# IDEA-CCNL/Fengshenbang-LM

Hardware: AMD Instinct MI355X
Metric: tokens/sec Ziya-LLaMA-13B ZeRO-3 (higher is better)
Workload: dtype bf16; 1 GPU; model=Ziya-LLaMA-13B, global_batch=16, micro_batch=16, seq_len=2048, parallelism=zero3_dp1, activation_checkpointing=True, ckpt_skip_interval=4

## Files before the change

fengshen_amd/ops/csrc/flash_attn.hip:

```cpp

#include "common.h"

typedef __attribute__((ext_vector_type(8))) short bf16x8;
typedef __attribute__((ext_vector_type(4))) float f32x4;

#define FA_QBLK 128
#define FA_KVBLK 64
#define FA_WAVES 8
#define FA_VPAD 8
#define FB_T 32

constexpr int fa_dpad(int d) { return (d + 31) / 32 * 32; }
constexpr int fa_swb(int dp) {
  int need = 2 * dp, p = 128;
  while (p < need) p <<= 1;
  return p;
}

__device__ __forceinline__ int kswz(int row, int byte_in_row) {
  return byte_in_row ^ ((row & 7) << 4);
}

__device__ __forceinline__ unsigned int fa_hash(unsigned long long seed,
                                                unsigned long long idx) {
// ... 800 lines not shown
    b, h, sq, sk, scale, dth, ksc, seed, stream); break;
  switch (d) {
    FWD_CASE(40) FWD_CASE(64) FWD_CASE(80)
    FWD_CASE(96) FWD_CASE(128) FWD_CASE(160)
  }
#undef FWD_CASE
}

template <int D>
static void launch_bwd(bool causal, const void* q, const void* k,
                       const void* v, const void* o, const void* dout,
                       const float* lse, void* dq, void* dk, void* dv,
                       float* delta_ws, const int* klens, int b, int h,
                       int sq, int sk, float scale, unsigned int dth,
                       float ksc, unsigned long long seed,
                       hipStream_t stream) {
  const long rows = (long)b * h * sq;
  {
    long blocks = (rows + 3) / 4;
    if (blocks > 4096) blocks = 4096;
    hipLaunchKernelGGL((flash_delta_kernel<D>), dim3((unsigned)blocks),
                       dim3(256), 0, stream, (const bf16_t*)dout,
                       (const bf16_t*)o, delta_ws, rows);
  }
  dim3 gq((sq + FA_QBLK - 1) / FA_QBLK, h, b);
  dim3 gkv((sk + FA_WAVES * 16 - 1) / (FA_WAVES * 16), h, b);
  dim3 block(FA_WAVES * 64);
  if (causal) {
    hipLaunchKernelGGL((flash_attn_bwd_dq_kernel<D, true>), gq, block, 0,
                       stream, (const bf16_t*)q, (const bf16_t*)k,
                       (const bf16_t*)v, (const bf16_t*)dout, lse, delta_ws,
                       (bf16_t*)dq, klens, b, h, sq, sk, scale, dth, ksc,
                       seed);
    hipLaunchKernelGGL((flash_attn_bwd_dkv_kernel<D, true>), gkv, block, 0,
                       stream, (const bf16_t*)q, (const bf16_t*)k,
                       (const bf16_t*)v, (const bf16_t*)dout, lse, delta_ws,
                       (bf16_t*)dk, (bf16_t*)dv, klens, b, h, sq, sk, scale,
                       dth, ksc, seed);
  } else {
    hipLaunchKernelGGL((flash_attn_bwd_dq_kernel<D, false>), gq, block, 0,
                       stream, (const bf16_t*)q, (const bf16_t*)k,
                       (const bf16_t*)v, (const bf16_t*)dout, lse, delta_ws,
                       (bf16_t*)dq, klens, b, h, sq, sk, scale, dth, ksc,
                       seed);
    hipLaunchKernelGGL((flash_attn_bwd_dkv_kernel<D, false>), gkv, block, 0,
                       stream, (const bf16_t*)q, (const bf16_t*)k,
                       (const bf16_t*)v, (const bf16_t*)dout, lse, delta_ws,
                       (bf16_t*)dk, (bf16_t*)dv, klens, b, h, sq, sk, scale,
                       dth, ksc, seed);
  }
}

extern "C" void fs_flash_attn_bwd(const void* q, const void* k, const void* v,
                                  const void* o, const void* dout,
                                  const float* lse, void* dq, void* dk,
                                  void* dv, float* delta_ws, const int* klens,
                                  int b, int h, int sq, int sk, int d,
                                  int causal, float scale, float drop_p,
                                  unsigned long long seed,
                                  hipStream_t stream) {
  const unsigned int dth =
      (drop_p > 0.f) ? (unsigned int)(drop_p * 4294967296.0) : 0u;
  const float ksc = (drop_p > 0.f) ? 1.f / (1.f - drop_p) : 1.f;
#define BWD_CASE(DD) case DD: launch_bwd<DD>(causal, q, k, v, o, dout, lse, \
    dq, dk, dv, delta_ws, klens, b, h, sq, sk, scale, dth, ksc, seed, \
    stream); break;
  switch (d) {
    BWD_CASE(40) BWD_CASE(64) BWD_CASE(80)
    BWD_CASE(96) BWD_CASE(128) BWD_CASE(160)
  }
#undef BWD_CASE
}


#define V3_QBLK 256
#define V3_KVBLK 64

typedef __attribute__((ext_vector_type(16))) float f32x16;

struct FaStrides {
  long b, h, r;
};

template <int D>
__global__ __launch_bounds__(256)
void flash_delta_v3_kernel(const bf16_t* __restrict__ dO,
                           const bf16_t* __restrict__ O,
                           float* __restrict__ delta, FaStrides dos,
                           FaStrides os, int h, int s) {
  const int lane = threadIdx.x & 63;
  const int wid = threadIdx.x >> 6;
  const bf16_t* dob = dO + blockIdx.z * dos.b + blockIdx.y * dos.h;
  const bf16_t* ob = O + blockIdx.z * os.b + blockIdx.y * os.h;
  float* dl = delta + ((long)blockIdx.z * h + blockIdx.y) * s;
  for (int row = blockIdx.x * 4 + wid; row < s; row += gridDim.x * 4) {
    const bf16_t* dop = dob + row * dos.r;
    const bf16_t* op = ob + row * os.r;
    float sacc = 0.f;
    for (int i = lane * 2; i < D; i += 128) {
#pragma unroll
      for (int j = 0; j < 2; ++j)
        sacc += __bfloat162float(dop[i + j]) * __bfloat162float(op[i + j]);
    }
    sacc = wave_reduce_sum(sacc);
    if (lane == 0) dl[row] = sacc;
  }
}

template <int D, bool CAUSAL, bool HAS_DROP>
__global__ __launch_bounds__(FA_WAVES * 64)
void flash_attn_fwd_v3_kernel(const bf16_t* __restrict__ Q,
                              const bf16_t* __restrict__ K,
                              const bf16_t* __restrict__ V,
                              bf16_t* __restrict__ O,
                              float* __restrict__ LSE,
                              const int* __restrict__ klens,
                              FaStrides qs, FaStrides os,
                              int b, int h, int s, float scale,
                              unsigned int drop_thresh, float keep_scale,
                              unsigned long long drop_seed) {
  constexpr int NC = D / 16;
  constexpr int NTO = D / 32;
  constexpr int SWB = fa_swb(D);

  __shared__ char k_raw[2][V3_KVBLK * SWB];
  __shared__ short vt_lds[2][D][V3_KVBLK + FA_VPAD];

  const int lane = threadIdx.x & 63;
  const int wave = threadIdx.x >> 6;
  const int hi = lane >> 5;
  const int ln = lane & 31;
  const long bh = (long)blockIdx.z * h + blockIdx.y;
  const long qoff = blockIdx.z * qs.b + blockIdx.y * qs.h;
  const bf16_t* Qp = Q + qoff;
  const bf16_t* Kp = K + qoff;
  const bf16_t* Vp = V + qoff;
  bf16_t* Op = O + blockIdx.z * os.b + blockIdx.y * os.h;

  const int klen = CAUSAL ? s : min(klens ? klens[blockIdx.z] : s, s);

  const int q0w = blockIdx.x * V3_QBLK + wave * 32;
  const bool q_active = q0w < s;
  const int q0c = q_active ? q0w : s - 32;
  const int my_q = q0c + ln;

  bf16x8 q_frag[NC];
#pragma unroll
  for (int c = 0; c < NC; ++c) {
    bf16x8 raw = *reinterpret_cast<const bf16x8*>(
        Qp + (long)my_q * qs.r + c * 16 + hi * 8);
#pragma unroll
    for (int j = 0; j < 8; ++j) {
      unsigned short u = (unsigned short)raw[j];
      float f = __uint_as_float(((unsigned int)u) << 16) * scale;
      raw[j] = fa_bf16bits(f);
    }
    q_frag[c] = raw;
  }

  float m_run = -INFINITY, l_run = 0.f;
  f32x16 o_acc[NTO];
#pragma unroll
  for (int t = 0; t < NTO; ++t) {
#pragma unroll
    for (int r = 0; r < 16; ++r) o_acc[t][r] = 0.f;
  }

  int n_kv_tiles;
  if (CAUSAL) {
    const int q_hi_row = min(blockIdx.x * V3_QBLK + V3_QBLK, s) - 1;
    n_kv_tiles = (q_hi_row / V3_KVBLK) + 1;
  } else {
    n_kv_tiles = (klen + V3_KVBLK - 1) / V3_KVBLK;
    if (n_kv_tiles < 1) n_kv_tiles = 1;
  }

  const int tid = threadIdx.x;
  constexpr int ELEMS = V3_KVBLK * D;
  constexpr int SWEEPS = (ELEMS + FA_WAVES * 64 * 8 - 1) / (FA_WAVES * 64 * 8);
  bf16x8 k_reg[SWEEPS], v_reg[SWEEPS];
#pragma unroll
  for (int sweep = 0; sweep < SWEEPS; ++sweep) {
    const int i = tid * 8 + sweep * (FA_WAVES * 64 * 8);
    if (i < ELEMS) {
      const long kr = min(i / D, s - 1);
      const int kc = i % D;
      k_reg[sweep] = *reinterpret_cast<const bf16x8*>(Kp + kr * qs.r + kc);
      v_reg[sweep] = *reinterpret_cast<const bf16x8*>(Vp + kr * qs.r + kc);
    }
  }

  {
#pragma unroll
    for (int sweep = 0; sweep < SWEEPS; ++sweep) {
      const int i = tid * 8 + sweep * (FA_WAVES * 64 * 8);
      if (i < ELEMS) {
        const int kr = i / D;
        const int kc = i % D;
        *reinterpret_cast<bf16x8*>(
            k_raw[0] + kr * SWB + kswz(kr, kc * 2)) = k_reg[sweep];
        bf16x8 vv = v_reg[sweep];
#pragma unroll
        for (int j = 0; j < 8; ++j)
          vt_lds[0][kc + j][kr ^ ((kc + j) & 0x38)] = vv[j];
      }
    }
  }
  int cur = 0;
  for (int kt = 0; kt < n_kv_tiles; ++kt) {
    const int k_base = kt * V3_KVBLK;
    __syncthreads();
    if (kt + 1 < n_kv_tiles) {
      const int nb = (kt + 1) * V3_KVBLK;
#pragma unroll
      for (int sweep = 0; sweep < SWEEPS; ++sweep) {
        const int i = tid * 8 + sweep * (FA_WAVES * 64 * 8);
        if (i < ELEMS) {
          const long kr = min((long)(nb + i / D), (long)s - 1);
          const int kc = i % D;
          k_reg[sweep] = *reinterpret_cast<const bf16x8*>(Kp + kr * qs.r + kc);
          v_reg[sweep] = *reinterpret_cast<const bf16x8*>(Vp + kr * qs.r + kc);
        }
      }
    }

    f32x16 st[2];
#pragma unroll
    for (int nt = 0; nt < 2; ++nt) {
#pragma unroll
      for (int r = 0; r < 16; ++r) st[nt][r] = 0.f;
    }
#pragma unroll
    for (int nt = 0; nt < 2; ++nt) {
      const int krow = nt * 32 + ln;
#pragma unroll
      for (int c = 0; c < NC; ++c) {
        bf16x8 a = *reinterpret_cast<const bf16x8*>(
            k_raw[cur] + krow * SWB + kswz(krow, (c * 16 + hi * 8) * 2));
        st[nt] = __builtin_amdgcn_mfma_f32_32x32x16_bf16(a, q_frag[c],
                                                         st[nt], 0, 0, 0);
      }
    }

    float p[32];
    float tmax = -INFINITY;
#pragma unroll
    for (int nt = 0; nt < 2; ++nt) {
#pragma unroll
      for (int r = 0; r < 16; ++r) {
        const int kcol = k_base + nt * 32 + (r & 3) + 8 * (r >> 2) + 4 * hi;
        float v = st[nt][r];
        if (CAUSAL ? (kcol > my_q) : (kcol >= klen)) v = -INFINITY;
        p[nt * 16 + r] = v;
        tmax = fmaxf(tmax, v);
      }
    }
    tmax = fmaxf(tmax, __shfl_xor(tmax, 32, 64));
    const float m_new = fmaxf(m_run, tmax);
    const float alpha = (m_run == -INFINITY) ? 0.f : __expf(m_run - m_new);
    const bool rescale = (m_new != m_run);
    m_run = m_new;
    float rs = 0.f;
#pragma unroll
    for (int i = 0; i < 32; ++i) {
      float e = (p[i] == -INFINITY) ? 0.f : __expf(p[i] - m_new);
      p[i] = e;
      rs += e;
    }
    rs += __shfl_xor(rs, 32, 64);
    l_run = l_run * alpha + rs;

    if (HAS_DROP && drop_thresh) {
      const unsigned long long qi =
          (bh * (unsigned long long)s + my_q) * (unsigned long long)s;
#pragma unroll
      for (int nt = 0; nt < 2; ++nt) {
#pragma unroll
        for (int r = 0; r < 16; ++r) {
          const int kcol =
              k_base + nt * 32 + (r & 3) + 8 * (r >> 2) + 4 * hi;
          float& pv = p[nt * 16 + r];
          pv = (fa_hash(drop_seed, qi + kcol) < drop_thresh)
                   ? 0.f : pv * keep_scale;
        }
      }
    }

    if (__any(rescale)) {
#pragma unroll
      for (int r = 0; r < 16; ++r) {
        const float al = __shfl(alpha, (r & 3) + 8 * (r >> 2) + 4 * hi, 64);
#pragma unroll
        for (int t = 0; t < NTO; ++t) o_acc[t][r] *= al;
      }
    }

    unsigned int pw[8][2];
#pragma unroll
    for (int G = 0; G < 8; ++G) {
      const int base = (G >> 2) * 16 + (G & 3) * 4;
#pragma unroll
      for (int k = 0; k < 2; ++k) {
        const unsigned int lo =
            (unsigned short)fa_bf16bits(p[base + 2 * k]);
        const unsigned int hi_b =
            (unsigned short)fa_bf16bits(p[base + 2 * k + 1]);
        pw[G][k] = (hi_b << 16) | lo;
      }
    }

#pragma unroll
    for (int c2 = 0; c2 < 4; ++c2) {
      unsigned int paw[4];
#pragma unroll
      for (int k = 0; k < 2; ++k) {
        auto pr = __builtin_amdgcn_permlane32_swap(
            (int)pw[2 * c2][k], (int)pw[2 * c2 + 1][k], false, false);
        paw[k] = (unsigned int)pr[0];
        paw[k + 2] = (unsigned int)pr[1];
      }
      bf16x8 pa;
#pragma unroll
      for (int k = 0; k < 4; ++k) {
        pa[2 * k] = (short)(paw[k] & 0xFFFF);
        pa[2 * k + 1] = (short)(paw[k] >> 16);
      }
#pragma unroll
      for (int t = 0; t < NTO; ++t) {
        const int dcol = t * 32 + ln;
        bf16x8 vb = *reinterpret_cast<const bf16x8*>(
            &vt_lds[cur][dcol][(c2 * 16 + hi * 8) ^ (dcol & 0x38)]);
        o_acc[t] = __builtin_amdgcn_mfma_f32_32x32x16_bf16(pa, vb, o_acc[t],
                                                           0, 0, 0);
      }
    }

    if (kt + 1 < n_kv_tiles) {
      const int nxt = cur ^ 1;
#pragma unroll
      for (int sweep = 0; sweep < SWEEPS; ++sweep) {
        const int i = tid * 8 + sweep * (FA_WAVES * 64 * 8);
        if (i < ELEMS) {
          const int kr = i / D;
          const int kc = i % D;
          *reinterpret_cast<bf16x8*>(
              k_raw[nxt] + kr * SWB + kswz(kr, kc * 2)) = k_reg[sweep];
          bf16x8 vv = v_reg[sweep];
#pragma unroll
          for (int j = 0; j < 8; ++j)
            vt_lds[nxt][kc + j][kr ^ ((kc + j) & 0x38)] = vv[j];
        }
      }
      cur = nxt;
    }
  }

  if (!q_active) return;
  const float my_inv_l = (l_run > 0.f) ? 1.f / l_run : 0.f;
#pragma unroll
  for (int r = 0; r < 16; ++r) {
    const int qrow = q0w + (r & 3) + 8 * (r >> 2) + 4 * hi;
    const float inv_l =
        __shfl(my_inv_l, (r & 3) + 8 * (r >> 2) + 4 * hi, 64);
#pragma unroll
    for (int t = 0; t < NTO; ++t) {
      Op[(long)qrow * os.r + t * 32 + ln] =
          __float2bfloat16(o_acc[t][r] * inv_l);
    }
  }
  if (hi == 0 && LSE) {
    LSE[bh * s + q0w + ln] = m_run + logf(fmaxf(l_run, 1e-30f));
  }
}

extern "C" void fs_flash_attn_fwd_v3_strided(
    const void* q, const void* k, const void* v, void* o, float* lse,
    const int* klens, const long* qs3, const long* os3, int b, int h, int s,
    int d, int causal, float scale, float drop_p, unsigned long long seed,
    hipStream_t stream) {
  const FaStrides qs{qs3[0], qs3[1], qs3[2]};
  const FaStrides os{os3[0], os3[1], os3[2]};
  dim3 grid((s + V3_QBLK - 1) / V3_QBLK, h, b);
  dim3 block(FA_WAVES * 64);
  const unsigned int dth =
      (drop_p > 0.f) ? (unsigned int)(drop_p * 4294967296.0) : 0u;
  const float ksc = (drop_p > 0.f) ? 1.f / (1.f - drop_p) : 1.f;
#define V3F(DD, CC, DR) hipLaunchKernelGGL( \
    (flash_attn_fwd_v3_kernel<DD, CC, DR>), \
    grid, block, 0, stream, (const bf16_t*)q, (const bf16_t*)k, \
    (const bf16_t*)v, (bf16_t*)o, lse, klens, qs, os, b, h, s, scale, dth, \
    ksc, seed)
  if (dth) {
    if (d == 128 && causal) V3F(128, true, true);
    else if (d == 128) V3F(128, false, true);
    else if (d == 96 && causal) V3F(96, true, true);
    else if (d == 96) V3F(96, false, true);
    else if (d == 64 && causal) V3F(64, true, true);
    else V3F(64, false, true);
  } else {
    if (d == 128 && causal) V3F(128, true, false);
    else if (d == 128) V3F(128, false, false);
    else if (d == 96 && causal) V3F(96, true, false);
    else if (d == 96) V3F(96, false, false);
    else if (d == 64 && causal) V3F(64, true, false);
    else V3F(64, false, false);
  }
#undef V3F
}

extern "C" void fs_flash_attn_fwd_v3(const void* q, const void* k,
                                     const void* v, void* o, float* lse,
                                     const int* klens, int b, int h, int s,
                                     int d, int causal, float scale,
                                     float drop_p, unsigned long long seed,
                                     hipStream_t stream) {
  const long c3[3] = {(long)h * s * d, (long)s * d, (long)d};
  fs_flash_attn_fwd_v3_strided(q, k, v, o, lse, klens, c3, c3, b, h, s, d,
                               causal, scale, drop_p, seed, stream);
}


#define B3_FB 32

template <int D, bool CAUSAL, bool HAS_DROP>
__global__ __launch_bounds__(FA_WAVES * 64)
void flash_attn_bwd_dq_v3_kernel(const bf16_t* __restrict__ Q,
                                 const bf16_t* __restrict__ K,
                                 const bf16_t* __restrict__ V,
                                 const bf16_t* __restrict__ dO,
                                 const float* __restrict__ LSE,
                                 const float* __restrict__ Delta,
                                 bf16_t* __restrict__ dQ,
                                 const int* __restrict__ klens,
                                 FaStrides qs, FaStrides dos, FaStrides gs,
                                 int b, int h, int s, float scale,
                                 unsigned int drop_thresh, float keep_scale,
                                 unsigned long long drop_seed) {
  constexpr int NC = D / 16;
  constexpr int NTO = D / 32;
  constexpr int SWB = fa_swb(D);

  __shared__ char k_raw[B3_FB * SWB];
  __shared__ char v_raw[B3_FB * SWB];
  __shared__ short kt_lds[D][B3_FB + FA_VPAD];
  __shared__ short p_x[FA_WAVES][32][B3_FB + FA_VPAD];

  const int lane = threadIdx.x & 63;
  const int wave = threadIdx.x >> 6;
  const int hi = lane >> 5;
  const int ln = lane & 31;
  const long bh = (long)blockIdx.z * h + blockIdx.y;
  const long qoff = blockIdx.z * qs.b + blockIdx.y * qs.h;
  const bf16_t* Qp = Q + qoff;
  const bf16_t* Kp = K + qoff;
  const bf16_t* Vp = V + qoff;
  const bf16_t* dOp = dO + blockIdx.z * dos.b + blockIdx.y * dos.h;
  bf16_t* dQp = dQ + blockIdx.z * gs.b + blockIdx.y * gs.h;
  const float* lse = LSE + bh * s;
  const float* dlt = Delta + bh * s;

  const int klen = CAUSAL ? s : min(klens ? klens[blockIdx.z] : s, s);
  const int q0w = blockIdx.x * V3_QBLK + wave * 32;
  const bool q_active = q0w < s;
  const int q0c = q_active ? q0w : s - 32;
  const int my_q = q0c + ln;

  bf16x8 q_frag[NC], do_frag[NC];
#pragma unroll
  for (int c = 0; c < NC; ++c) {
    bf16x8 raw = *reinterpret_cast<const bf16x8*>(
        Qp + (long)my_q * qs.r + c * 16 + hi * 8);
#pragma unroll
    for (int j = 0; j < 8; ++j) {
      unsigned short u = (unsigned short)raw[j];
      raw[j] = fa_bf16bits(
          __uint_as_float(((unsigned int)u) << 16) * scale);
    }
    q_frag[c] = raw;
    do_frag[c] = *reinterpret_cast<const bf16x8*>(
        dOp + (long)my_q * dos.r + c * 16 + hi * 8);
  }
  const float lse_r = lse[my_q];
  const float dlt_r = dlt[my_q];

  f32x16 dq_acc[NTO];
#pragma unroll
  for (int t = 0; t < NTO; ++t) {
#pragma unroll
    for (int r = 0; r < 16; ++r) dq_acc[t][r] = 0.f;
  }

  int n_kv_tiles;
  if (CAUSAL) {
    const int q_hi_row = min(blockIdx.x * V3_QBLK + V3_QBLK, s) - 1;
    n_kv_tiles = (q_hi_row / B3_FB) + 1;
  } else {
    n_kv_tiles = (klen + B3_FB - 1) / B3_FB;
  }

  for (int kt = 0; kt < n_kv_tiles; ++kt) {
    const int k_base = kt * B3_FB;
    __syncthreads();
    {
      const int tid = threadIdx.x;
      for (int i = tid * 8; i < B3_FB * D; i += FA_WAVES * 64 * 8) {
        const int kr = i / D;
        const int kc = i % D;
        const long krg = min(k_base + kr, s - 1);
        bf16x8 kk = *reinterpret_cast<const bf16x8*>(Kp + krg * qs.r + kc);
        *reinterpret_cast<bf16x8*>(k_raw + kr * SWB + kswz(kr, kc * 2)) = kk;
        bf16x8 vv = *reinterpret_cast<const bf16x8*>(Vp + krg * qs.r + kc);
        *reinterpret_cast<bf16x8*>(v_raw + kr * SWB + kswz(kr, kc * 2)) = vv;
#pragma unroll
        for (int j = 0; j < 8; ++j)
          kt_lds[kc + j][kr ^ ((kc + j) & 0x18)] = kk[j];
      }
    }
    __syncthreads();

    f32x16 st, dpt;
#pragma unroll
    for (int r = 0; r < 16; ++r) {
      st[r] = 0.f;
      dpt[r] = 0.f;
    }
    {
      const int krow = ln;
#pragma unroll
      for (int c = 0; c < NC; ++c) {
        bf16x8 ka = *reinterpret_cast<const bf16x8*>(
            k_raw + krow * SWB + kswz(krow, (c * 16 + hi * 8) * 2));
        st = __builtin_amdgcn_mfma_f32_32x32x16_bf16(ka, q_frag[c], st,
                                                     0, 0, 0);
        bf16x8 va = *reinterpret_cast<const bf16x8*>(
            v_raw + krow * SWB + kswz(krow, (c * 16 + hi * 8) * 2));
        dpt = __builtin_amdgcn_mfma_f32_32x32x16_bf16(va, do_frag[c], dpt,
                                                      0, 0, 0);
      }
    }

#pragma unroll
    for (int g = 0; g < 4; ++g) {
      short pk[4] __attribute__((aligned(8)));
#pragma unroll
      for (int j = 0; j < 4; ++j) {
        const int r = g * 4 + j;
        const int kcol = k_base + (r & 3) + 8 * (r >> 2) + 4 * hi;
        const bool masked = CAUSAL ? (kcol > my_q) : (kcol >= klen);
        float pv = masked ? 0.f : __expf(st[r] - lse_r);
        float dpv = dpt[r];
        if (HAS_DROP && drop_thresh) {
          const unsigned long long idx =
              (bh * (unsigned long long)s + my_q) *
                  (unsigned long long)s + kcol;
          dpv = (fa_hash(drop_seed, idx) < drop_thresh)
                    ? 0.f : dpv * keep_scale;
        }
        pk[j] = fa_bf16bits(pv * (dpv - dlt_r) * scale);
      }
      *reinterpret_cast<long*>(&p_x[wave][ln][8 * g + 4 * hi]) =
          *reinterpret_cast<const long*>(pk);
    }
    __builtin_amdgcn_s_waitcnt(0);

#pragma unroll
    for (int c2 = 0; c2 < 2; ++c2) {
      bf16x8 pa = *reinterpret_cast<const bf16x8*>(
          &p_x[wave][ln][c2 * 16 + hi * 8]);
#pragma unroll
      for (int t = 0; t < NTO; ++t) {
        const int dcol = t * 32 + ln;
        bf16x8 kb = *reinterpret_cast<const bf16x8*>(
            &kt_lds[dcol][(c2 * 16 + hi * 8) ^ (dcol & 0x18)]);
        dq_acc[t] = __builtin_amdgcn_mfma_f32_32x32x16_bf16(pa, kb,
                                                            dq_acc[t],
                                                            0, 0, 0);
      }
    }
  }

  if (!q_active) return;
#pragma unroll
  for (int r = 0; r < 16; ++r) {
    const int qrow = q0w + (r & 3) + 8 * (r >> 2) + 4 * hi;
#pragma unroll
    for (int t = 0; t < NTO; ++t)
      dQp[(long)qrow * gs.r + t * 32 + ln] = __float2bfloat16(dq_acc[t][r]);
  }
}

template <int D, bool CAUSAL, bool HAS_DROP>
__global__ __launch_bounds__(FA_WAVES * 64)
void flash_attn_bwd_dkv_v3_kernel(const bf16_t* __restrict__ Q,
                                  const bf16_t* __restrict__ K,
                                  const bf16_t* __restrict__ V,
                                  const bf16_t* __restrict__ dO,
                                  const float* __restrict__ LSE,
                                  const float* __restrict__ Delta,
                                  bf16_t* __restrict__ dK,
                                  bf16_t* __restrict__ dV,
                                  const int* __restrict__ klens,
                                  FaStrides qs, FaStrides dos, FaStrides gs,
                                  int b, int h, int s, float scale,
                                  unsigned int drop_thresh, float keep_scale,
                                  unsigned long long drop_seed) {
  constexpr int NC = D / 16;
  constexpr int NTO = D / 32;
  constexpr int SWB = fa_swb(D);

  __shared__ char q_raw[B3_FB * SWB];
  __shared__ char do_raw[B3_FB * SWB];
  __shared__ short qt_lds[D][B3_FB + FA_VPAD];
  __shared__ short dot_lds[D][B3_FB + FA_VPAD];
  __shared__ short p_x[FA_WAVES][32][B3_FB + FA_VPAD];
  __shared__ short ds_x[FA_WAVES][32][B3_FB + FA_VPAD];

  const int lane = threadIdx.x & 63;
  const int wave = threadIdx.x >> 6;
  const int hi = lane >> 5;
  const int ln = lane & 31;
  const long bh = (long)blockIdx.z * h + blockIdx.y;
  const long qoff = blockIdx.z * qs.b + blockIdx.y * qs.h;
  const bf16_t* Qp = Q + qoff;
  const bf16_t* Kp = K + qoff;
  const bf16_t* Vp = V + qoff;
  const bf16_t* dOp = dO + blockIdx.z * dos.b + blockIdx.y * dos.h;
  const long goff = blockIdx.z * gs.b + blockIdx.y * gs.h;
  bf16_t* dKp = dK + goff;
  bf16_t* dVp = dV + goff;
  const float* lse = LSE + bh * s;
  const float* dlt = Delta + bh * s;

  const int klen = CAUSAL ? s : min(klens ? klens[blockIdx.z] : s, s);
  const int kv0_blk = blockIdx.x * V3_QBLK;
  const int kv0w = kv0_blk + wave * 32;
  const bool kv_active = kv0w < s;
  const int kv0c = kv_active ? kv0w : s - 32;
  const int my_kv = kv0c + ln;

  f32x16 dv_acc[NTO], dk_acc[NTO];
#pragma unroll
  for (int t = 0; t < NTO; ++t) {
#pragma unroll
    for (int r = 0; r < 16; ++r) {
      dv_acc[t][r] = 0.f;
      dk_acc[t][r] = 0.f;
    }
  }

  const int first_qt = CAUSAL ? kv0_blk / B3_FB : 0;
  const int n_q_tiles = s / B3_FB;

  for (int qt = first_qt; qt < n_q_tiles; ++qt) {
    const int q_base = qt * B3_FB;
    __syncthreads();
    {
      const int tid = threadIdx.x;
      for (int i = tid * 8; i < B3_FB * D; i += FA_WAVES * 64 * 8) {
        const int qr = i / D;
        const int qc = i % D;
        bf16x8 qq = *reinterpret_cast<const bf16x8*>(
            Qp + (long)(q_base + qr) * qs.r + qc);
        *reinterpret_cast<bf16x8*>(q_raw + qr * SWB + kswz(qr, qc * 2)) = qq;
        bf16x8 dd = *reinterpret_cast<const bf16x8*>(
            dOp + (long)(q_base + qr) * dos.r + qc);
        *reinterpret_cast<bf16x8*>(do_raw + qr * SWB + kswz(qr, qc * 2)) =
            dd;
#pragma unroll
        for (int j = 0; j < 8; ++j) {
          qt_lds[qc + j][qr ^ ((qc + j) & 0x18)] = qq[j];
          dot_lds[qc + j][qr ^ ((qc + j) & 0x18)] = dd[j];
        }
      }
    }
    __syncthreads();

    f32x16 st;
#pragma unroll
    for (int r = 0; r < 16; ++r) st[r] = 0.f;
#pragma unroll
    for (int c = 0; c < NC; ++c) {
      bf16x8 ka = *reinterpret_cast<const bf16x8*>(
          Kp + (long)my_kv * qs.r + c * 16 + hi * 8);
      bf16x8 qb = *reinterpret_cast<const bf16x8*>(
          q_raw + ln * SWB + kswz(ln, (c * 16 + hi * 8) * 2));
      st = __builtin_amdgcn_mfma_f32_32x32x16_bf16(ka, qb, st, 0, 0, 0);
    }
    f32x16 dpt;
#pragma unroll
    for (int r = 0; r < 16; ++r) dpt[r] = 0.f;
#pragma unroll
    for (int c = 0; c < NC; ++c) {
      bf16x8 va = *reinterpret_cast<const bf16x8*>(
          Vp + (long)my_kv * qs.r + c * 16 + hi * 8);
      bf16x8 db = *reinterpret_cast<const bf16x8*>(
          do_raw + ln * SWB + kswz(ln, (c * 16 + hi * 8) * 2));
      dpt = __builtin_amdgcn_mfma_f32_32x32x16_bf16(va, db, dpt, 0, 0, 0);
    }

    const int qcol = q_base + ln;
    const float lse_c = lse[qcol];
    const float dlt_c = dlt[qcol];

#pragma unroll
    for (int r = 0; r < 16; ++r) {
      const int kvrow_loc = (r & 3) + 8 * (r >> 2) + 4 * hi;
      const int kvrow = kv0c + kvrow_loc;
      const bool masked = CAUSAL ? (qcol < kvrow) : (kvrow >= klen);
      float pv = masked ? 0.f : __expf(st[r] * scale - lse_c);
      float dm = 1.f;
      if (HAS_DROP && drop_thresh) {
        const unsigned long long idx =
            (bh * (unsigned long long)s + qcol) *
                (unsigned long long)s + kvrow;
        dm = (fa_hash(drop_seed, idx) < drop_thresh) ? 0.f : keep_scale;
      }
      p_x[wave][kvrow_loc][ln] = fa_bf16bits(pv * dm);
      ds_x[wave][kvrow_loc][ln] =
          fa_bf16bits(pv * (dm * dpt[r] - dlt_c) * scale);
    }
    __builtin_amdgcn_s_waitcnt(0);

#pragma unroll
    for (int c2 = 0; c2 < 2; ++c2) {
      bf16x8 pa = *reinterpret_cast<const bf16x8*>(
          &p_x[wave][ln][c2 * 16 + hi * 8]);
#pragma unroll
      for (int t = 0; t < NTO; ++t) {
        const int dcol = t * 32 + ln;
        bf16x8 bfrag = *reinterpret_cast<const bf16x8*>(
            &dot_lds[dcol][(c2 * 16 + hi * 8) ^ (dcol & 0x18)]);
        dv_acc[t] = __builtin_amdgcn_mfma_f32_32x32x16_bf16(
            pa, bfrag, dv_acc[t], 0, 0, 0);
      }
    }

#pragma unroll
    for (int c2 = 0; c2 < 2; ++c2) {
      bf16x8 pa = *reinterpret_cast<const bf16x8*>(
          &ds_x[wave][ln][c2 * 16 + hi * 8]);
#pragma unroll
      for (int t = 0; t < NTO; ++t) {
        const int dcol = t * 32 + ln;
        bf16x8 bfrag = *reinterpret_cast<const bf16x8*>(
            &qt_lds[dcol][(c2 * 16 + hi * 8) ^ (dcol & 0x18)]);
        dk_acc[t] = __builtin_amdgcn_mfma_f32_32x32x16_bf16(
            pa, bfrag, dk_acc[t], 0, 0, 0);
      }
    }
  }

  if (!kv_active) return;
#pragma unroll
  for (int r = 0; r < 16; ++r) {
    const int kvrow = kv0w + (r & 3) + 8 * (r >> 2) + 4 * hi;
#pragma unroll
    for (int t = 0; t < NTO; ++t) {
      dKp[(long)kvrow * gs.r + t * 32 + ln] = __float2bfloat16(dk_acc[t][r]);
      dVp[(long)kvrow * gs.r + t * 32 + ln] = __float2bfloat16(dv_acc[t][r]);
    }
  }
}

template <int D, bool CAUSAL, bool HAS_DROP>
static void launch_bwd_v3(const void* q, const void* k, const void* v,
                          const void* o, const void* dout, const float* lse,
                          void* dq, void* dk, void* dv, float* delta_ws,
                          const int* klens, FaStrides qs, FaStrides os,
                          FaStrides dos, FaStrides gs, int b, int h, int s,
                          float scale, unsigned int dth, float ksc,
                          unsigned long long seed, hipStream_t stream) {
  {
    int bx = (s + 31) / 32;
    if (bx > 16) bx = 16;
    hipLaunchKernelGGL((flash_delta_v3_kernel<D>), dim3(bx, h, b), dim3(256),
                       0, stream, (const bf16_t*)dout, (const bf16_t*)o,
                       delta_ws, dos, os, h, s);
  }
  dim3 grid((s + V3_QBLK - 1) / V3_QBLK, h, b);
  dim3 block(FA_WAVES * 64);
  hipLaunchKernelGGL((flash_attn_bwd_dq_v3_kernel<D, CAUSAL, HAS_DROP>),
                     grid, block, 0, stream, (const bf16_t*)q,
                     (const bf16_t*)k, (const bf16_t*)v, (const bf16_t*)dout,
                     lse, delta_ws, (bf16_t*)dq, klens, qs, dos, gs, b, h, s,
                     scale, dth, ksc, seed);
  hipLaunchKernelGGL((flash_attn_bwd_dkv_v3_kernel<D, CAUSAL, HAS_DROP>),
                     grid, block, 0, stream, (const bf16_t*)q,
                     (const bf16_t*)k, (const bf16_t*)v, (const bf16_t*)dout,
                     lse, delta_ws, (bf16_t*)dk, (bf16_t*)dv, klens, qs, dos,
                     gs, b, h, s, scale, dth, ksc, seed);
}

extern "C" void fs_flash_attn_bwd_v3_strided(
    const void* q, const void* k, const void* v, const void* o,
    const void* dout, const float* lse, void* dq, void* dk, void* dv,
    float* delta_ws, const int* klens, const long* qs3, const long* os3,
    const long* dos3, const long* gs3, int b, int h, int s, int d,
    int causal, float scale, float drop_p, unsigned long long seed,
    hipStream_t stream) {
  const FaStrides qs{qs3[0], qs3[1], qs3[2]};
  const FaStrides os{os3[0], os3[1], os3[2]};
  const FaStrides dos{dos3[0], dos3[1], dos3[2]};
  const FaStrides gs{gs3[0], gs3[1], gs3[2]};
  const unsigned int dth =
      (drop_p > 0.f) ? (unsigned int)(drop_p * 4294967296.0) : 0u;
  const float ksc = (drop_p > 0.f) ? 1.f / (1.f - drop_p) : 1.f;
#define BWD3(DD, CC, DR) launch_bwd_v3<DD, CC, DR>( \
      q, k, v, o, dout, lse, dq, dk, dv, delta_ws, klens, qs, os, dos, gs, \
      b, h, s, scale, dth, ksc, seed, stream)
  if (dth) {
    if (d == 128 && causal) BWD3(128, true, true);
    else if (d == 128) BWD3(128, false, true);
    else if (d == 96 && causal) BWD3(96, true, true);
    else if (d == 96) BWD3(96, false, true);
    else if (d == 64 && causal) BWD3(64, true, true);
    else BWD3(64, false, true);
  } else {
    if (d == 128 && causal) BWD3(128, true, false);
    else if (d == 128) BWD3(128, false, false);
    else if (d == 96 && causal) BWD3(96, true, false);
    else if (d == 96) BWD3(96, false, false);
    else if (d == 64 && causal) BWD3(64, true, false);
    else BWD3(64, false, false);
  }
#undef BWD3
}

extern "C" void fs_flash_attn_bwd_v3(const void* q, const void* k,
// ... 14 lines not shown
```

Before: 9889 tokens/s.

## Use LDS transpose reads in flash-attention v3 kernels instead of transposed copies

Stores V (forward) and K/Q/dO (backward) in LDS only in row-major swizzled form and reads the transposed MFMA B-operand fragments with ds_read_tr16_b64. This drops the scalar element-by-element transpose stores into separate transposed LDS arrays. The change also skips fully masked causal KV tiles per wave, double-buffers K/V in the dQ kernel with register prefetch, and hoists K/V fragments out of the q-tile loop in the dK/dV kernel. It depends on new swizzle/address math and the gfx950 transpose-read builtin being correct, and it narrows the LDS waitcnt.

```diff
diff --git a/fengshen_amd/ops/csrc/flash_attn.hip b/fengshen_amd/ops/csrc/flash_attn.hip
--- a/fengshen_amd/ops/csrc/flash_attn.hip
+++ b/fengshen_amd/ops/csrc/flash_attn.hip
@@ -906,6 +906,45 @@
   long b, h, r;
 };
 
+typedef __attribute__((ext_vector_type(4))) short bf16x4;
+typedef __attribute__((address_space(3))) bf16x4 lds_bf16x4;
+
+template <int SWB>
+__device__ __forceinline__ int v3_off(int row, int ch) {
+  static_assert(SWB == 256 || SWB == 128, "row stride");
+  if (SWB == 256)
+    return 256 * row + 16 * (ch ^ (((row & 3) << 2) | ((row >> 2) & 3)));
+  return 128 * row + 16 * (ch ^ ((((row >> 1) & 1) << 2) | ((row >> 2) & 3)));
+}
+
+template <int SWB>
+__device__ __forceinline__ int v3_tr_addr(int lane, int row0, int col0) {
+  const int i = lane & 15;
+  const int col = col0 + 16 * ((lane >> 4) & 1) + 4 * (i & 3);
+  return v3_off<SWB>(row0 + (i >> 2), col >> 3) + 2 * (col & 7);
+}
+
+__device__ __forceinline__ bf16x8 v3_tr_frag(const char* a0, const char* a1) {
+  const bf16x4 lo = __builtin_amdgcn_ds_read_tr16_b64_v4i16((lds_bf16x4*)a0);
+  const bf16x4 hi = __builtin_amdgcn_ds_read_tr16_b64_v4i16((lds_bf16x4*)a1);
+  return __builtin_shufflevector(lo, hi, 0, 1, 2, 3, 4, 5, 6, 7);
+}
+
+template <int SWB>
+__device__ __forceinline__ bf16x8 v3_tr_bfrag(const char* rows, int tbase,
+                                              int t) {
+  const int a0 = tbase ^ (64 * t);
+  return v3_tr_frag(rows + a0, rows + (a0 ^ 16) + 4 * SWB);
+}
+
+__device__ __forceinline__ void v3_wait_lds() {
+  __builtin_amdgcn_s_waitcnt(0xC07F);
+}
+
+__device__ __forceinline__ int dkv_xoff(int row, int u) {
+  return 64 * row + 8 * (u ^ ((row >> 1) & 7));
+}
+
 template <int D>
 __global__ __launch_bounds__(256)
 void flash_delta_v3_kernel(const bf16_t* __restrict__ dO,
@@ -947,8 +986,10 @@
   constexpr int NTO = D / 32;
   constexpr int SWB = fa_swb(D);
 
-  __shared__ char k_raw[2][V3_KVBLK * SWB];
-  __shared__ short vt_lds[2][D][V3_KVBLK + FA_VPAD];
+  __shared__ __attribute__((aligned(16)))
+  char k_raw[2][V3_KVBLK * SWB];
+  __shared__ __attribute__((aligned(16)))
+  char v_raw[2][V3_KVBLK * SWB];
 
   const int lane = threadIdx.x & 63;
   const int wave = threadIdx.x >> 6;
@@ -1023,13 +1064,14 @@
         const int kc = i % D;
         *reinterpret_cast<bf16x8*>(
             k_raw[0] + kr * SWB + kswz(kr, kc * 2)) = k_reg[sweep];
-        bf16x8 vv = v_reg[sweep];
-#pragma unroll
-        for (int j = 0; j < 8; ++j)
-          vt_lds[0][kc + j][kr ^ ((kc + j) & 0x38)] = vv[j];
-      }
-    }
-  }
+        *reinterpret_cast<bf16x8*>(
+            v_raw[0] + v3_off<SWB>(kr, kc >> 3)) = v_reg[sweep];
+      }
+    }
+  }
+  const int v_tr = v3_tr_addr<SWB>(lane, 8 * hi, 0);
+  const int q_last_w = __builtin_amdgcn_readfirstlane(q0c) + 31;
+
   int cur = 0;
   for (int kt = 0; kt < n_kv_tiles; ++kt) {
     const int k_base = kt * V3_KVBLK;
@@ -1048,114 +1090,115 @@
       }
     }
 
-    f32x16 st[2];
-#pragma unroll
-    for (int nt = 0; nt < 2; ++nt) {
-#pragma unroll
-      for (int r = 0; r < 16; ++r) st[nt][r] = 0.f;
-    }
-#pragma unroll
-    for (int nt = 0; nt < 2; ++nt) {
-      const int krow = nt * 32 + ln;
-#pragma unroll
-      for (int c = 0; c < NC; ++c) {
-        bf16x8 a = *reinterpret_cast<const bf16x8*>(
-            k_raw[cur] + krow * SWB + kswz(krow, (c * 16 + hi * 8) * 2));
-        st[nt] = __builtin_amdgcn_mfma_f32_32x32x16_bf16(a, q_frag[c],
-                                                         st[nt], 0, 0, 0);
-      }
-    }
-
-    float p[32];
-    float tmax = -INFINITY;
-#pragma unroll
-    for (int nt = 0; nt < 2; ++nt) {
-#pragma unroll
-      for (int r = 0; r < 16; ++r) {
-        const int kcol = k_base + nt * 32 + (r & 3) + 8 * (r >> 2) + 4 * hi;
-        float v = st[nt][r];
-        if (CAUSAL ? (kcol > my_q) : (kcol >= klen)) v = -INFINITY;
-        p[nt * 16 + r] = v;
-        tmax = fmaxf(tmax, v);
-      }
-    }
-    tmax = fmaxf(tmax, __shfl_xor(tmax, 32, 64));
-    const float m_new = fmaxf(m_run, tmax);
-    const float alpha = (m_run == -INFINITY) ? 0.f : __expf(m_run - m_new);
-    const bool rescale = (m_new != m_run);
-    m_run = m_new;
-    float rs = 0.f;
-#pragma unroll
-    for (int i = 0; i < 32; ++i) {
-      float e = (p[i] == -INFINITY) ? 0.f : __expf(p[i] - m_new);
-      p[i] = e;
-      rs += e;
-    }
-    rs += __shfl_xor(rs, 32, 64);
-    l_run = l_run * alpha + rs;
-
-    if (HAS_DROP && drop_thresh) {
-      const unsigned long long qi =
-          (bh * (unsigned long long)s + my_q) * (unsigned long long)s;
+    if (!CAUSAL || k_base <= q_last_w) {
+      f32x16 st[2];
 #pragma unroll
       for (int nt = 0; nt < 2; ++nt) {
 #pragma unroll
+        for (int r = 0; r < 16; ++r) st[nt][r] = 0.f;
+      }
+#pragma unroll
+      for (int nt = 0; nt < 2; ++nt) {
+        const int krow = nt * 32 + ln;
+#pragma unroll
+        for (int c = 0; c < NC; ++c) {
+          bf16x8 a = *reinterpret_cast<const bf16x8*>(
+              k_raw[cur] + krow * SWB + kswz(krow, (c * 16 + hi * 8) * 2));
+          st[nt] = __builtin_amdgcn_mfma_f32_32x32x16_bf16(a, q_frag[c],
+                                                           st[nt], 0, 0, 0);
+        }
+      }
+
+      float p[32];
+      float tmax = -INFINITY;
+#pragma unroll
+      for (int nt = 0; nt < 2; ++nt) {
+#pragma unroll
         for (int r = 0; r < 16; ++r) {
-          const int kcol =
-              k_base + nt * 32 + (r & 3) + 8 * (r >> 2) + 4 * hi;
-          float& pv = p[nt * 16 + r];
-          pv = (fa_hash(drop_seed, qi + kcol) < drop_thresh)
-                   ? 0.f : pv * keep_scale;
-        }
-      }
-    }
-
-    if (__any(rescale)) {
-#pragma unroll
-      for (int r = 0; r < 16; ++r) {
-        const float al = __shfl(alpha, (r & 3) + 8 * (r >> 2) + 4 * hi, 64);
-#pragma unroll
-        for (int t = 0; t < NTO; ++t) o_acc[t][r] *= al;
-      }
-    }
-
-    unsigned int pw[8][2];
-#pragma unroll
-    for (int G = 0; G < 8; ++G) {
-      const int base = (G >> 2) * 16 + (G & 3) * 4;
-#pragma unroll
-      for (int k = 0; k < 2; ++k) {
-        const unsigned int lo =
-            (unsigned short)fa_bf16bits(p[base + 2 * k]);
-        const unsigned int hi_b =
-            (unsigned short)fa_bf16bits(p[base + 2 * k + 1]);
-        pw[G][k] = (hi_b << 16) | lo;
-      }
-    }
-
-#pragma unroll
-    for (int c2 = 0; c2 < 4; ++c2) {
-      unsigned int paw[4];
-#pragma unroll
-      for (int k = 0; k < 2; ++k) {
-        auto pr = __builtin_amdgcn_permlane32_swap(
-            (int)pw[2 * c2][k], (int)pw[2 * c2 + 1][k], false, false);
-        paw[k] = (unsigned int)pr[0];
-        paw[k + 2] = (unsigned int)pr[1];
-      }
-      bf16x8 pa;
-#pragma unroll
-      for (int k = 0; k < 4; ++k) {
-        pa[2 * k] = (short)(paw[k] & 0xFFFF);
-        pa[2 * k + 1] = (short)(paw[k] >> 16);
-      }
-#pragma unroll
-      for (int t = 0; t < NTO; ++t) {
-        const int dcol = t * 32 + ln;
-        bf16x8 vb = *reinterpret_cast<const bf16x8*>(
-            &vt_lds[cur][dcol][(c2 * 16 + hi * 8) ^ (dcol & 0x38)]);
-        o_acc[t] = __builtin_amdgcn_mfma_f32_32x32x16_bf16(pa, vb, o_acc[t],
-                                                           0, 0, 0);
+          const int kcol = k_base + nt * 32 + (r & 3) + 8 * (r >> 2) + 4 * hi;
+          float v = st[nt][r];
+          if (CAUSAL ? (kcol > my_q) : (kcol >= klen)) v = -INFINITY;
+          p[nt * 16 + r] = v;
+          tmax = fmaxf(tmax, v);
+        }
+      }
+      tmax = fmaxf(tmax, __shfl_xor(tmax, 32, 64));
+      const float m_new = fmaxf(m_run, tmax);
+      const float alpha = (m_run == -INFINITY) ? 0.f : __expf(m_run - m_new);
+      const bool rescale = (m_new != m_run);
+      m_run = m_new;
+      float rs = 0.f;
+#pragma unroll
+      for (int i = 0; i < 32; ++i) {
+        float e = (p[i] == -INFINITY) ? 0.f : __expf(p[i] - m_new);
+        p[i] = e;
+        rs += e;
+      }
+      rs += __shfl_xor(rs, 32, 64);
+      l_run = l_run * alpha + rs;
+
+      if (HAS_DROP && drop_thresh) {
+        const unsigned long long qi =
+            (bh * (unsigned long long)s + my_q) * (unsigned long long)s;
+#pragma unroll
+        for (int nt = 0; nt < 2; ++nt) {
+#pragma unroll
+          for (int r = 0; r < 16; ++r) {
+            const int kcol =
+                k_base + nt * 32 + (r & 3) + 8 * (r >> 2) + 4 * hi;
+            float& pv = p[nt * 16 + r];
+            pv = (fa_hash(drop_seed, qi + kcol) < drop_thresh)
+                     ? 0.f : pv * keep_scale;
+          }
+        }
+      }
+
+      if (__any(rescale)) {
+#pragma unroll
+        for (int r = 0; r < 16; ++r) {
+          const float al = __shfl(alpha, (r & 3) + 8 * (r >> 2) + 4 * hi, 64);
+#pragma unroll
+          for (int t = 0; t < NTO; ++t) o_acc[t][r] *= al;
+        }
+      }
+
+      unsigned int pw[8][2];
+#pragma unroll
+      for (int G = 0; G < 8; ++G) {
+        const int base = (G >> 2) * 16 + (G & 3) * 4;
+#pragma unroll
+        for (int k = 0; k < 2; ++k) {
+          const unsigned int lo =
+              (unsigned short)fa_bf16bits(p[base + 2 * k]);
+          const unsigned int hi_b =
+              (unsigned short)fa_bf16bits(p[base + 2 * k + 1]);
+          pw[G][k] = (hi_b << 16) | lo;
+        }
+      }
+
+#pragma unroll
+      for (int c2 = 0; c2 < 4; ++c2) {
+        unsigned int paw[4];
+#pragma unroll
+        for (int k = 0; k < 2; ++k) {
+          auto pr = __builtin_amdgcn_permlane32_swap(
+              (int)pw[2 * c2][k], (int)pw[2 * c2 + 1][k], false, false);
+          paw[k] = (unsigned int)pr[0];
+          paw[k + 2] = (unsigned int)pr[1];
+        }
+        bf16x8 pa;
+#pragma unroll
+        for (int k = 0; k < 4; ++k) {
+          pa[2 * k] = (short)(paw[k] & 0xFFFF);
+          pa[2 * k + 1] = (short)(paw[k] >> 16);
+        }
+#pragma unroll
+        for (int t = 0; t < NTO; ++t) {
+          const char* vrow = v_raw[cur] + c2 * 16 * SWB;
+          bf16x8 vb = v3_tr_bfrag<SWB>(vrow, v_tr, t);
+          o_acc[t] = __builtin_amdgcn_mfma_f32_32x32x16_bf16(pa, vb, o_acc[t],
+                                                             0, 0, 0);
+        }
       }
     }
 
@@ -1169,10 +1212,8 @@
           const int kc = i % D;
           *reinterpret_cast<bf16x8*>(
               k_raw[nxt] + kr * SWB + kswz(kr, kc * 2)) = k_reg[sweep];
-          bf16x8 vv = v_reg[sweep];
-#pragma unroll
-          for (int j = 0; j < 8; ++j)
-            vt_lds[nxt][kc + j][kr ^ ((kc + j) & 0x38)] = vv[j];
+          *reinterpret_cast<bf16x8*>(
+              v_raw[nxt] + v3_off<SWB>(kr, kc >> 3)) = v_reg[sweep];
         }
       }
       cur = nxt;
@@ -1264,9 +1305,8 @@
   constexpr int NTO = D / 32;
   constexpr int SWB = fa_swb(D);
 
-  __shared__ char k_raw[B3_FB * SWB];
-  __shared__ char v_raw[B3_FB * SWB];
-  __shared__ short kt_lds[D][B3_FB + FA_VPAD];
+  __shared__ __attribute__((aligned(16))) char k_raw[2][B3_FB * SWB];
+  __shared__ __attribute__((aligned(16))) char v_raw[2][B3_FB * SWB];
   __shared__ short p_x[FA_WAVES][32][B3_FB + FA_VPAD];
 
   const int lane = threadIdx.x & 63;
@@ -1322,83 +1362,99 @@
     n_kv_tiles = (klen + B3_FB - 1) / B3_FB;
   }
 
+  const int st_i = threadIdx.x * 8;
+  const bool st_on = st_i < B3_FB * D;
+  const int st_r = st_on ? st_i / D : 0;
+  const int st_c = st_on ? st_i % D : 0;
+  const int st_off = v3_off<SWB>(st_r, st_c >> 3);
+  bf16x8 k_reg, v_reg;
+  {
+    const long krg = min(st_r, s - 1);
+    k_reg = *reinterpret_cast<const bf16x8*>(Kp + krg * qs.r + st_c);
+    v_reg = *reinterpret_cast<const bf16x8*>(Vp + krg * qs.r + st_c);
+  }
+  if (st_on) {
+    *reinterpret_cast<bf16x8*>(k_raw[0] + st_off) = k_reg;
+    *reinterpret_cast<bf16x8*>(v_raw[0] + st_off) = v_reg;
+  }
+  const int k_tr = v3_tr_addr<SWB>(lane, 8 * hi, 0);
+  const int kv_row = v3_off<SWB>(ln, hi);
+  const int q_last_w = __builtin_amdgcn_readfirstlane(q0c) + 31;
+
+  int cur = 0;
   for (int kt = 0; kt < n_kv_tiles; ++kt) {
     const int k_base = kt * B3_FB;
     __syncthreads();
-    {
-      const int tid = threadIdx.x;
-      for (int i = tid * 8; i < B3_FB * D; i += FA_WAVES * 64 * 8) {
-        const int kr = i / D;
-        const int kc = i % D;
-        const long krg = min(k_base + kr, s - 1);
-        bf16x8 kk = *reinterpret_cast<const bf16x8*>(Kp + krg * qs.r + kc);
-        *reinterpret_cast<bf16x8*>(k_raw + kr * SWB + kswz(kr, kc * 2)) = kk;
-        bf16x8 vv = *reinterpret_cast<const bf16x8*>(Vp + krg * qs.r + kc);
-        *reinterpret_cast<bf16x8*>(v_raw + kr * SWB + kswz(kr, kc * 2)) = vv;
-#pragma unroll
-        for (int j = 0; j < 8; ++j)
-          kt_lds[kc + j][kr ^ ((kc + j) & 0x18)] = kk[j];
-      }
-    }
-    __syncthreads();
-
-    f32x16 st, dpt;
-#pragma unroll
-    for (int r = 0; r < 16; ++r) {
-      st[r] = 0.f;
-      dpt[r] = 0.f;
-    }
-    {
-      const int krow = ln;
-#pragma unroll
-      for (int c = 0; c < NC; ++c) {
-        bf16x8 ka = *reinterpret_cast<const bf16x8*>(
-            k_raw + krow * SWB + kswz(krow, (c * 16 + hi * 8) * 2));
-        st = __builtin_amdgcn_mfma_f32_32x32x16_bf16(ka, q_frag[c], st,
-                                                     0, 0, 0);
-        bf16x8 va = *reinterpret_cast<const bf16x8*>(
-            v_raw + krow * SWB + kswz(krow, (c * 16 + hi * 8) * 2));
-        dpt = __builtin_amdgcn_mfma_f32_32x32x16_bf16(va, do_frag[c], dpt,
-                                                      0, 0, 0);
-      }
-    }
-
-#pragma unroll
-    for (int g = 0; g < 4; ++g) {
-      short pk[4] __attribute__((aligned(8)));
-#pragma unroll
-      for (int j = 0; j < 4; ++j) {
-        const int r = g * 4 + j;
-        const int kcol = k_base + (r & 3) + 8 * (r >> 2) + 4 * hi;
-        const bool masked = CAUSAL ? (kcol > my_q) : (kcol >= klen);
-        float pv = masked ? 0.f : __expf(st[r] - lse_r);
-        float dpv = dpt[r];
-        if (HAS_DROP && drop_thresh) {
-          const unsigned long long idx =
-              (bh * (unsigned long long)s + my_q) *
-                  (unsigned long long)s + kcol;
-          dpv = (fa_hash(drop_seed, idx) < drop_thresh)
-                    ? 0.f : dpv * keep_scale;
-        }
-        pk[j] = fa_bf16bits(pv * (dpv - dlt_r) * scale);
-      }
-      *reinterpret_cast<long*>(&p_x[wave][ln][8 * g + 4 * hi]) =
-          *reinterpret_cast<const long*>(pk);
-    }
-    __builtin_amdgcn_s_waitcnt(0);
-
-#pragma unroll
-    for (int c2 = 0; c2 < 2; ++c2) {
-      bf16x8 pa = *reinterpret_cast<const bf16x8*>(
-          &p_x[wave][ln][c2 * 16 + hi * 8]);
-#pragma unroll
-      for (int t = 0; t < NTO; ++t) {
-        const int dcol = t * 32 + ln;
-        bf16x8 kb = *reinterpret_cast<const bf16x8*>(
-            &kt_lds[dcol][(c2 * 16 + hi * 8) ^ (dcol & 0x18)]);
-        dq_acc[t] = __builtin_amdgcn_mfma_f32_32x32x16_bf16(pa, kb,
-                                                            dq_acc[t],
-                                                            0, 0, 0);
+    if (kt + 1 < n_kv_tiles) {
+      const long krg = min(k_base + B3_FB + st_r, s - 1);
+      k_reg = *reinterpret_cast<const bf16x8*>(Kp + krg * qs.r + st_c);
+      v_reg = *reinterpret_cast<const bf16x8*>(Vp + krg * qs.r + st_c);
+    }
+
+    if (!CAUSAL || k_base <= q_last_w) {
+      f32x16 st, dpt;
+#pragma unroll
+      for (int r = 0; r < 16; ++r) {
+        st[r] = 0.f;
+        dpt[r] = 0.f;
+      }
+      {
+#pragma unroll
+        for (int c = 0; c < NC; ++c) {
+          const int roff = kv_row ^ (32 * c);
+          bf16x8 ka = *reinterpret_cast<const bf16x8*>(k_raw[cur] + roff);
+          st = __builtin_amdgcn_mfma_f32_32x32x16_bf16(ka, q_frag[c], st,
+                                                       0, 0, 0);
+          bf16x8 va = *reinterpret_cast<const bf16x8*>(v_raw[cur] + roff);
+          dpt = __builtin_amdgcn_mfma_f32_32x32x16_bf16(va, do_frag[c], dpt,
+                                                        0, 0, 0);
+        }
+      }
+
+#pragma unroll
+      for (int g = 0; g < 4; ++g) {
+        short pk[4] __attribute__((aligned(8)));
+#pragma unroll
+        for (int j = 0; j < 4; ++j) {
+          const int r = g * 4 + j;
+          const int kcol = k_base + (r & 3) + 8 * (r >> 2) + 4 * hi;
+          const bool masked = CAUSAL ? (kcol > my_q) : (kcol >= klen);
+          float pv = masked ? 0.f : __expf(st[r] - lse_r);
+          float dpv = dpt[r];
+          if (HAS_DROP && drop_thresh) {
+            const unsigned long long idx =
+                (bh * (unsigned long long)s + my_q) *
+                    (unsigned long long)s + kcol;
+            dpv = (fa_hash(drop_seed, idx) < drop_thresh)
+                      ? 0.f : dpv * keep_scale;
+          }
+          pk[j] = fa_bf16bits(pv * (dpv - dlt_r) * scale);
+        }
+        *reinterpret_cast<long*>(&p_x[wave][ln][8 * g + 4 * hi]) =
+            *reinterpret_cast<const long*>(pk);
+      }
+      v3_wait_lds();
+
+#pragma unroll
+      for (int c2 = 0; c2 < 2; ++c2) {
+        bf16x8 pa = *reinterpret_cast<const bf16x8*>(
+            &p_x[wave][ln][c2 * 16 + hi * 8]);
+        const char* krows = k_raw[cur] + c2 * 16 * SWB;
+#pragma unroll
+        for (int t = 0; t < NTO; ++t) {
+          bf16x8 kb = v3_tr_bfrag<SWB>(krows, k_tr, t);
+          dq_acc[t] = __builtin_amdgcn_mfma_f32_32x32x16_bf16(pa, kb,
+                                                              dq_acc[t],
+                                                              0, 0, 0);
+        }
+      }
+    }
+
+    if (kt + 1 < n_kv_tiles) {
+      cur ^= 1;
+      if (st_on) {
+        *reinterpret_cast<bf16x8*>(k_raw[cur] + st_off) = k_reg;
+        *reinterpret_cast<bf16x8*>(v_raw[cur] + st_off) = v_reg;
       }
     }
   }
@@ -1432,12 +1488,10 @@
   constexpr int NTO = D / 32;
   constexpr int SWB = fa_swb(D);
 
-  __shared__ char q_raw[B3_FB * SWB];
-  __shared__ char do_raw[B3_FB * SWB];
-  __shared__ short qt_lds[D][B3_FB + FA_VPAD];
-  __shared__ short dot_lds[D][B3_FB + FA_VPAD];
-  __shared__ short p_x[FA_WAVES][32][B3_FB + FA_VPAD];
-  __shared__ short ds_x[FA_WAVES][32][B3_FB + FA_VPAD];
+  __shared__ __attribute__((aligned(16))) char q_raw[B3_FB * SWB];
+  __shared__ __attribute__((aligned(16))) char do_raw[B3_FB * SWB];
+  __shared__ __attribute__((aligned(16))) char p_x[FA_WAVES][32 * 64];
+  __shared__ __attribute__((aligned(16))) char ds_x[FA_WAVES][32 * 64];
 
   const int lane = threadIdx.x & 63;
   const int wave = threadIdx.x >> 6;
@@ -1475,85 +1529,104 @@
   const int first_qt = CAUSAL ? kv0_blk / B3_FB : 0;
   const int n_q_tiles = s / B3_FB;
 
+  const int st_i = threadIdx.x * 8;
+  const bool st_on = st_i < B3_FB * D;
+  const int st_r = st_on ? st_i / D : 0;
+  const int st_c = st_on ? st_i % D : 0;
+  const int st_off = v3_off<SWB>(st_r, st_c >> 3);
+  const int qd_tr = v3_tr_addr<SWB>(lane, 8 * hi, 0);
+  const int qd_row = v3_off<SWB>(ln, hi);
+  int x_tr[2];
+#pragma unroll
+  for (int e = 0; e < 2; ++e) {
+    const int i = lane & 15;
+    const int row = 8 * hi + 4 * e + (i >> 2);
+    x_tr[e] = dkv_xoff(row, 4 * ((lane >> 4) & 1) + (i & 3));
+  }
+  bf16x8 k_frag[NC], v_frag[NC];
+#pragma unroll
+  for (int c = 0; c < NC; ++c) {
+    k_frag[c] = *reinterpret_cast<const bf16x8*>(
+        Kp + (long)my_kv * qs.r + c * 16 + hi * 8);
+    v_frag[c] = *reinterpret_cast<const bf16x8*>(
+        Vp + (long)my_kv * qs.r + c * 16 + hi * 8);
+  }
+
   for (int qt = first_qt; qt < n_q_tiles; ++qt) {
     const int q_base = qt * B3_FB;
     __syncthreads();
     {
-      const int tid = threadIdx.x;
-      for (int i = tid * 8; i < B3_FB * D; i += FA_WAVES * 64 * 8) {
-        const int qr = i / D;
-        const int qc = i % D;
-        bf16x8 qq = *reinterpret_cast<const bf16x8*>(
-            Qp + (long)(q_base + qr) * qs.r + qc);
-        *reinterpret_cast<bf16x8*>(q_raw + qr * SWB + kswz(qr, qc * 2)) = qq;
-        bf16x8 dd = *reinterpret_cast<const bf16x8*>(
-            dOp + (long)(q_base + qr) * dos.r + qc);
-        *reinterpret_cast<bf16x8*>(do_raw + qr * SWB + kswz(qr, qc * 2)) =
-            dd;
-#pragma unroll
-        for (int j = 0; j < 8; ++j) {
-          qt_lds[qc + j][qr ^ ((qc + j) & 0x18)] = qq[j];
-          dot_lds[qc + j][qr ^ ((qc + j) & 0x18)] = dd[j];
-        }
-      }
-    }
-    __syncthreads();
-
-    f32x16 st;
-#pragma unroll
-    for (int r = 0; r < 16; ++r) st[r] = 0.f;
-#pragma unroll
-    for (int c = 0; c < NC; ++c) {
-      bf16x8 ka = *reinterpret_cast<const bf16x8*>(
-          Kp + (long)my_kv * qs.r + c * 16 + hi * 8);
-      bf16x8 qb = *reinterpret_cast<const bf16x8*>(
-          q_raw + ln * SWB + kswz(ln, (c * 16 + hi * 8) * 2));
-      st = __builtin_amdgcn_mfma_f32_32x32x16_bf16(ka, qb, st, 0, 0, 0);
-    }
-    f32x16 dpt;
-#pragma unroll
-    for (int r = 0; r < 16; ++r) dpt[r] = 0.f;
-#pragma unroll
-    for (int c = 0; c < NC; ++c) {
-      bf16x8 va = *reinterpret_cast<const bf16x8*>(
-          Vp + (long)my_kv * qs.r + c * 16 + hi * 8);
-      bf16x8 db = *reinterpret_cast<const bf16x8*>(
-          do_raw + ln * SWB + kswz(ln, (c * 16 + hi * 8) * 2));
-      dpt = __builtin_amdgcn_mfma_f32_32x32x16_bf16(va, db, dpt, 0, 0, 0);
-    }
-
+      const long qrg = q_base + st_r;
+      const bf16x8 qq =
+          *reinterpret_cast<const bf16x8*>(Qp + qrg * qs.r + st_c);
+      const bf16x8 dd =
+          *reinterpret_cast<const bf16x8*>(dOp + qrg * dos.r + st_c);
+      if (st_on) {
+        *reinterpret_cast<bf16x8*>(q_raw + st_off) = qq;
+        *reinterpret_cast<bf16x8*>(do_raw + st_off) = dd;
+      }
+    }
     const int qcol = q_base + ln;
     const float lse_c = lse[qcol];
     const float dlt_c = dlt[qcol];
-
-#pragma unroll
-    for (int r = 0; r < 16; ++r) {
-      const int kvrow_loc = (r & 3) + 8 * (r >> 2) + 4 * hi;
-      const int kvrow = kv0c + kvrow_loc;
-      const bool masked = CAUSAL ? (qcol < kvrow) : (kvrow >= klen);
-      float pv = masked ? 0.f : __expf(st[r] * scale - lse_c);
-      float dm = 1.f;
-      if (HAS_DROP && drop_thresh) {
-        const unsigned long long idx =
-            (bh * (unsigned long long)s + qcol) *
-                (unsigned long long)s + kvrow;
-        dm = (fa_hash(drop_seed, idx) < drop_thresh) ? 0.f : keep_scale;
-      }
-      p_x[wave][kvrow_loc][ln] = fa_bf16bits(pv * dm);
-      ds_x[wave][kvrow_loc][ln] =
-          fa_bf16bits(pv * (dm * dpt[r] - dlt_c) * scale);
-    }
-    __builtin_amdgcn_s_waitcnt(0);
+    __syncthreads();
+
+    f32x16 st, dpt;
+#pragma unroll
+    for (int r = 0; r < 16; ++r) st[r] = 0.f;
+#pragma unroll
+    for (int c = 0; c < NC; ++c) {
+      bf16x8 qb = *reinterpret_cast<const bf16x8*>(
+          q_raw + (qd_row ^ (32 * c)));
+      st = __builtin_amdgcn_mfma_f32_32x32x16_bf16(k_frag[c], qb, st, 0, 0,
+                                                   0);
+    }
+#pragma unroll
+    for (int r = 0; r < 16; ++r) dpt[r] = 0.f;
+#pragma unroll
+    for (int c = 0; c < NC; ++c) {
+      bf16x8 db = *reinterpret_cast<const bf16x8*>(
+          do_raw + (qd_row ^ (32 * c)));
+      dpt = __builtin_amdgcn_mfma_f32_32x32x16_bf16(v_frag[c], db, dpt, 0, 0,
+                                                    0);
+    }
+
+#pragma unroll
+    for (int g = 0; g < 4; ++g) {
+      short pk[4] __attribute__((aligned(8)));
+      short dk4[4] __attribute__((aligned(8)));
+#pragma unroll
+      for (int j = 0; j < 4; ++j) {
+        const int r = g * 4 + j;
+        const int kvrow = kv0c + (r & 3) + 8 * (r >> 2) + 4 * hi;
+        const bool masked = CAUSAL ? (qcol < kvrow) : (kvrow >= klen);
+        float pv = masked ? 0.f : __expf(st[r] * scale - lse_c);
+        float dm = 1.f;
+        if (HAS_DROP && drop_thresh) {
+          const unsigned long long idx =
+              (bh * (unsigned long long)s + qcol) *
+                  (unsigned long long)s + kvrow;
+          dm = (fa_hash(drop_seed, idx) < drop_thresh) ? 0.f : keep_scale;
+        }
+        pk[j] = fa_bf16bits(pv * dm);
+        dk4[j] = fa_bf16bits(pv * (dm * dpt[r] - dlt_c) * scale);
+      }
+      const int xo = dkv_xoff(ln, 2 * g + hi);
+      *reinterpret_cast<long*>(p_x[wave] + xo) =
+          *reinterpret_cast<const long*>(pk);
+      *reinterpret_cast<long*>(ds_x[wave] + xo) =
+          *reinterpret_cast<const long*>(dk4);
+    }
+    v3_wait_lds();
 
 #pragma unroll
     for (int c2 = 0; c2 < 2; ++c2) {
-      bf16x8 pa = *reinterpret_cast<const bf16x8*>(
-          &p_x[wave][ln][c2 * 16 + hi * 8]);
+      bf16x8 pa = v3_tr_frag(p_x[wave] + c2 * 16 * 64 + x_tr[0],
+                             p_x[wave] + c2 * 16 * 64 + x_tr[1]);
+      const char* drows = do_raw + c2 * 16 * SWB;
 #pragma unroll
       for (int t = 0; t < NTO; ++t) {
-        const int dcol = t * 32 + ln;
-        bf16x8 bfrag = *reinterpret_cast<const bf16x8*>(
-            &dot_lds[dcol][(c2 * 16 + hi * 8) ^ (dcol & 0x18)]);
+        bf16x8 bfrag = v3_tr_bfrag<SWB>(drows, qd_tr, t);
         dv_acc[t] = __builtin_amdgcn_mfma_f32_32x32x16_bf16(
             pa, bfrag, dv_acc[t], 0, 0, 0);
       }
@@ -1561,13 +1634,12 @@
 
 #pragma unroll
     for (int c2 = 0; c2 < 2; ++c2) {
-      bf16x8 pa = *reinterpret_cast<const bf16x8*>(
-          &ds_x[wave][ln][c2 * 16 + hi * 8]);
+      bf16x8 pa = v3_tr_frag(ds_x[wave] + c2 * 16 * 64 + x_tr[0],
+                             ds_x[wave] + c2 * 16 * 64 + x_tr[1]);
+      const char* qrows = q_raw + c2 * 16 * SWB;
 #pragma unroll
       for (int t = 0; t < NTO; ++t) {
-        const int dcol = t * 32 + ln;
-        bf16x8 bfrag = *reinterpret_cast<const bf16x8*>(
-            &qt_lds[dcol][(c2 * 16 + hi * 8) ^ (dcol & 0x18)]);
+        bf16x8 bfrag = v3_tr_bfrag<SWB>(qrows, qd_tr, t);
         dk_acc[t] = __builtin_amdgcn_mfma_f32_32x32x16_bf16(
             pa, bfrag, dk_acc[t], 0, 0, 0);
       }
```

Result: faster. 10220 tokens/s (median of 6 runs) (+3.3%).
